# Pointcept/Pointcept

Measured on AMD Instinct MI355X. Metric: scenes/sec (fwd+bwd+optimizer) PTv3 ScanNet-semseg @ ~100k pts, higher is better.
Workload: dtype bf16; 1 GPU; PT-v3m1 base (46.2M params) + seg head + CE + Lovasz, fwd+bwd+AdamW, 8 scenes x 102400 voxels per GPU, patch 1024, 4 orders; global_batch=8, parallelism=dp1, params=46167572, amp=bf16 autocast, points_per_gpu=819200, loss=CrossEntropy(ignore_index=-1) + LovaszSoftmax

## Files before the change

### pointcept_amd/csrc/attention.hip

```cpp
#include "ptc_common.h"
#include <stdlib.h>

typedef __attribute__((ext_vector_type(8))) short s16x8;
typedef __attribute__((ext_vector_type(4))) short s16x4;
typedef __attribute__((ext_vector_type(16))) float f32x16;
typedef __bf16 bf16x2_t __attribute__((ext_vector_type(2)));
typedef float f32x2_t __attribute__((ext_vector_type(2)));

#define AT_WAVES 8
#define AT_THREADS (AT_WAVES * 64)
#define AT_MAX_L 1024
#define AT_MIN_WAVES 4
#define AT_LOG2E 1.4426950408889634f
#define AT_LN2 0.6931471805599453f
#ifndef AT_SPLIT_BELOW
#define AT_SPLIT_BELOW 2048
#endif
#define AT_FIXED_REF_MAX 64.0f

__device__ __forceinline__ uint32_t pack_bf16x2(float lo, float hi) {
  f32x2_t f = {lo, hi};
  bf16x2_t h = __builtin_convertvector(f, bf16x2_t);
  return *reinterpret_cast<uint32_t*>(&h);
}
// ... 389 lines not shown
      if (kt < n_tiles) {
        expo(s1, pb);
        ldv();
        pv(pa);
        ldv();
        pv(pb);
      } else {
        ldv();
        pv(pa);
      }
    } else {
      float m = -INFINITY;
      const unsigned char* kp = kbase;
      const unsigned char* vp = vbase;
      for (int kt = 0; kt < n_tiles; ++kt) {
        const s16x8 kf = *reinterpret_cast<const s16x8*>(kp);
        kp += 1024;
        f32x16 s = mfma32(kf, qhi, zero16());
        s = mfma32(kf, qlo, s);
        if (kt == n_tiles - 1 && L < Lp) {
#pragma unroll
          for (int r = 0; r < 16; ++r)
            if (kt * 32 + crow(r, h2) >= L) s[r] = -INFINITY;
        }
        float mt = s[0];
#pragma unroll
        for (int r = 1; r < 16; ++r) mt = fmaxf(mt, s[r]);
        mt = fmaxf(mt, __shfl_xor(mt, 32, 64));
        const float m_new = fmaxf(m, mt);
        const float alpha = __builtin_amdgcn_exp2f(m - m_new);
        m = m_new;
#pragma unroll
        for (int r = 0; r < 9; ++r) acc[r] *= alpha;
        uint32_t pk[8];
#pragma unroll
        for (int i = 0; i < 8; ++i)
          pk[i] = pack_bf16x2(__builtin_amdgcn_exp2f(s[2 * i] - m), __builtin_amdgcn_exp2f(s[2 * i + 1] - m));
#pragma unroll
        for (int mm = 0; mm < 2; ++mm) {
          const s16x8 pf = make_frag(pk[4 * mm], pk[4 * mm + 1], pk[4 * mm + 2], pk[4 * mm + 3]);
          const s16x8 vf = *reinterpret_cast<const s16x8*>(vp + mm * voff);
          acc = mfma32(vf, pf, acc);
        }
        vp += vstride;
      }
      ref2 = m;
    }
    const float l = __shfl(acc[8], col, 64);
    const float inv = 1.f / l;
    if (q < L) {
      uint16_t* o = out + ((int64_t)(a + q) * H + head) * 16;
      uint2 w0, w1;
      w0.x = at_out<F16>(pack_bf16x2(acc[0] * inv, acc[1] * inv)); w0.y = at_out<F16>(pack_bf16x2(acc[2] * inv, acc[3] * inv));
      w1.x = at_out<F16>(pack_bf16x2(acc[4] * inv, acc[5] * inv)); w1.y = at_out<F16>(pack_bf16x2(acc[6] * inv, acc[7] * inv));
      *reinterpret_cast<uint2*>(o + 4 * h2) = w0;
      *reinterpret_cast<uint2*>(o + 8 + 4 * h2) = w1;
      if (h2 == 0) lse[(int64_t)head * total + a + q] = ref2 * AT_LN2 + __logf(l);
    }
  }
}


__device__ __forceinline__ int at_krow(int g) { return 16 * (g & 1) + 4 * (g >> 1); }
struct TrAddr16 { int lo, hi; };
__device__ __forceinline__ TrAddr16 tr_addr16(int lane) {
  const int lp = lane & 15, g = lane >> 4;
  const int row = at_krow(g) + (lp >> 2), cq = lp & 3;
  TrAddr16 a;
  a.lo = rm_off(row, cq >> 1) + ((cq & 1) << 3);
  a.hi = rm_off(row + 8, cq >> 1) + ((cq & 1) << 3);
  return a;
}
__device__ __forceinline__ void at_to_b16(uint32_t (&pk)[8], s16x8& lo, s16x8& hi) {
#pragma unroll
  for (int j = 0; j < 4; ++j) at_swap16(pk[j], pk[4 + j]);
  lo = make_frag(pk[0], pk[1], pk[2], pk[3]);
  hi = make_frag(pk[4], pk[5], pk[6], pk[7]);
}

template <int LP, bool F16>
__global__ void __launch_bounds__(AT_THREADS, AT_MIN_WAVES)
attn_bwd_dq_kernel(const uint16_t* __restrict__ qkv, const uint16_t* __restrict__ out, const uint16_t* __restrict__ dout,
                   const float* __restrict__ lse, const int32_t* __restrict__ cu, int H, float scale, int64_t total,
                   int lp_max, int n_units, int qs, uint16_t* __restrict__ dqkv, float* __restrict__ delta) {
  extern __shared__ __attribute__((aligned(16))) unsigned char smem[];
  const int lunit = at_unit(n_units * qs);
  if (lunit >= n_units * qs) return;
  const int unit = lunit / qs, part = lunit - unit * qs;
  const int seq = unit / H, head = unit % H;
  const int a = cu[seq], L = cu[seq + 1] - a;
  if (L <= 0) return;
  const int Lp = (L + 31) & ~31, n_tiles = Lp >> 5;
  if (Lp > lp_max) {
    if (part == 0) at_poison_rows<F16>(dqkv + qkv_off(a, 0, H, head), (int64_t)3 * H * 16, L, nullptr);
    return;
  }
  const int t_per = (n_tiles + qs - 1) / qs, t_lo = part * t_per, t_hi = (t_lo + t_per) < n_tiles ? (t_lo + t_per) : n_tiles;
  if (t_lo >= n_tiles) return;
  unsigned char* Vsm = smem;
  unsigned char* Ksm = smem + (size_t)lp_max * 32;
  const int64_t rs = (int64_t)3 * H * 16;
  stage_row_major<F16>(qkv + qkv_off(a, 2, H, head), rs, L, Lp, Vsm);
  stage_row_major<F16>(qkv + qkv_off(a, 1, H, head), rs, L, Lp, Ksm);
  __syncthreads();

  const int lane = ptc_lane(), wave = threadIdx.x >> 6;
  const int col = lane & 31, h2 = lane >> 5;
  const float c = scale * AT_LOG2E;
  const TrAddr16 ta = tr_addr16(lane);
  const int rmo = rm_off(col, h2);

  for (int qt = t_lo + wave; qt < t_hi; qt += AT_WAVES) {
    const int q = qt * 32 + col;
    const bool qv = q < L;
    const s16x8 qf = ld_global_frag<F16>(qkv + qkv_off(a + q, 0, H, head) + h2 * 8, qv);
    const int64_t orow = ((int64_t)(a + q) * H + head) * 16 + h2 * 8;
    const s16x8 dof = ld_global_frag<F16>(dout + orow, qv);
    const s16x8 of = ld_global_frag<F16>(out + orow, qv);
    float dl = 0.f;
#pragma unroll
    for (int j = 0; j < 8; ++j) dl += bf16_bits_to_float((uint16_t)dof[j]) * bf16_bits_to_float((uint16_t)of[j]);
    dl += __shfl_xor(dl, 32, 64);
    const float l2 = qv ? lse[(int64_t)head * total + a + q] * AT_LOG2E : INFINITY;
    if (qv && h2 == 0) delta[(int64_t)head * total + a + q] = dl;
    s16x8 qhi, qlo;
    split_scaled(qf, c, qhi, qlo);
    const f32x16 negl = splat16(-l2), negd = splat16(-dl);
    at_f32x4 acc0 = {0.f, 0.f, 0.f, 0.f}, acc1 = {0.f, 0.f, 0.f, 0.f};
    {
      const int KOFF = LP ? LP * 32 : lp_max * 32;
      const unsigned char* pv = Vsm + rmo;
      const unsigned char* pl = Ksm + ta.lo;
      const unsigned char* ph = Ksm + ta.hi;
      auto tile = [&](const int o) {
        const s16x8 vf = *reinterpret_cast<const s16x8*>(pv + o);
        const s16x8 kf = *reinterpret_cast<const s16x8*>(pv + o + KOFF);
        f32x16 s = mfma32(kf, qhi, negl);
        s = mfma32(kf, qlo, s);
        const f32x16 dp = mfma32(vf, dof, negd);
        uint32_t pk[8];
#pragma unroll
        for (int i = 0; i < 8; ++i)
          pk[i] = pack_bf16x2(__builtin_amdgcn_exp2f(s[2 * i]) * dp[2 * i], __builtin_amdgcn_exp2f(s[2 * i + 1]) * dp[2 * i + 1]);
        s16x8 ds0, ds1;
        at_to_b16(pk, ds0, ds1);
        const s16x8 ktf = ld_tr_pair(pl + o, ph + o);
        acc0 = mfma16(ktf, ds0, acc0);
        acc1 = mfma16(ktf, ds1, acc1);
      };
      int kt = 0;
      for (; kt + 1 < n_tiles; kt += 2) {
        tile(0);
        tile(1024);
        pv += 2048; pl += 2048; ph += 2048;
      }
      if (kt < n_tiles) tile(0);
    }
    const int g = lane >> 4, n = lane & 15;
#pragma unroll
    for (int t = 0; t < 2; ++t) {
      const int qq = qt * 32 + 16 * t + n;
      if (qq < L) {
        const at_f32x4 v = t ? acc1 : acc0;
        uint2 w;
        w.x = at_out<F16>(pack_bf16x2(v[0] * scale, v[1] * scale));
        w.y = at_out<F16>(pack_bf16x2(v[2] * scale, v[3] * scale));
        *reinterpret_cast<uint2*>(dqkv + qkv_off(a + qq, 0, H, head) + 4 * g) = w;
      }
    }
  }
}

#define AT_PAD_LSE 1.0e30f
template <int LP, bool F16>
__global__ void __launch_bounds__(AT_THREADS, AT_MIN_WAVES)
attn_bwd_dkv_kernel(const uint16_t* __restrict__ qkv, const uint16_t* __restrict__ dout, const float* __restrict__ lse,
                    const float* __restrict__ delta, const int32_t* __restrict__ cu, int H, float scale, int64_t total,
                    int lp_max, int n_units, int qs, uint16_t* __restrict__ dqkv) {
  extern __shared__ __attribute__((aligned(16))) unsigned char smem[];
  const int lunit = at_unit(n_units * qs);
  if (lunit >= n_units * qs) return;
  const int unit = lunit / qs, part = lunit - unit * qs;
  const int seq = unit / H, head = unit % H;
  const int a = cu[seq], L = cu[seq + 1] - a;
  if (L <= 0) return;
  const int Lp = (L + 31) & ~31, n_tiles = Lp >> 5;
  if (Lp > lp_max) {
    if (part == 0) {
      at_poison_rows<F16>(dqkv + qkv_off(a, 1, H, head), (int64_t)3 * H * 16, L, nullptr);
      at_poison_rows<F16>(dqkv + qkv_off(a, 2, H, head), (int64_t)3 * H * 16, L, nullptr);
    }
    return;
  }
  const int t_per = (n_tiles + qs - 1) / qs, t_lo = part * t_per, t_hi = (t_lo + t_per) < n_tiles ? (t_lo + t_per) : n_tiles;
  if (t_lo >= n_tiles) return;
  unsigned char* Qsm = smem;
  float* nl = reinterpret_cast<float*>(smem + (size_t)lp_max * 64);
  float* nd = nl + lp_max;
  stage_row_major<F16>(qkv + qkv_off(a, 0, H, head), (int64_t)3 * H * 16, L, Lp, Qsm);
  stage_row_major<F16>(dout + ((int64_t)a * H + head) * 16, (int64_t)H * 16, L, Lp, smem + (size_t)lp_max * 32);
  for (int q = threadIdx.x; q < Lp; q += AT_THREADS) {
    nl[q] = q < L ? -lse[(int64_t)head * total + a + q] * AT_LOG2E : -AT_PAD_LSE;
    nd[q] = q < L ? -delta[(int64_t)head * total + a + q] : 0.f;
  }
  __syncthreads();

  const int lane = ptc_lane(), wave = threadIdx.x >> 6;
  const int col = lane & 31, h2 = lane >> 5;
  const float c = scale * AT_LOG2E;
  const TrAddr16 ta = tr_addr16(lane);
  const int rmo = rm_off(col, h2);

  for (int kt = t_lo + wave; kt < t_hi; kt += AT_WAVES) {
    const int key = kt * 32 + col;
    const s16x8 kf = ld_global_frag<F16>(qkv + qkv_off(a + key, 1, H, head) + h2 * 8, key < L);
    const s16x8 vf = ld_global_frag<F16>(qkv + qkv_off(a + key, 2, H, head) + h2 * 8, key < L);
    s16x8 khi, klo;
    split_scaled(kf, c, khi, klo);
    at_f32x4 dv0 = {0.f, 0.f, 0.f, 0.f}, dv1 = dv0, dk0 = dv0, dk1 = dv0;
    {
      const int DOFF = LP ? LP * 32 : lp_max * 32, NOFF = (LP ? LP : lp_max) * 4;
      const unsigned char* pq = Qsm + rmo;
      const unsigned char* pl = Qsm + ta.lo;
      const unsigned char* ph = Qsm + ta.hi;
      const unsigned char* pc = reinterpret_cast<const unsigned char*>(nl) + 16 * h2;
      auto tile = [&](const int o, const int oc) {
        const s16x8 qf = *reinterpret_cast<const s16x8*>(pq + o);
        const s16x8 dof = *reinterpret_cast<const s16x8*>(pq + o + DOFF);
        f32x16 s, dp;
#pragma unroll
        for (int r4 = 0; r4 < 4; ++r4) {
          const at_f32x4 l4 = *reinterpret_cast<const at_f32x4*>(pc + oc + 32 * r4);
          const at_f32x4 d4 = *reinterpret_cast<const at_f32x4*>(pc + oc + 32 * r4 + NOFF);
#pragma unroll
          for (int e = 0; e < 4; ++e) { s[4 * r4 + e] = l4[e]; dp[4 * r4 + e] = d4[e]; }
        }
        s = mfma32(qf, khi, s);
        s = mfma32(qf, klo, s);
        dp = mfma32(dof, vf, dp);
        uint32_t pp[8], ps[8];
#pragma unroll
        for (int i = 0; i < 8; ++i) {
          const float p0 = __builtin_amdgcn_exp2f(s[2 * i]), p1 = __builtin_amdgcn_exp2f(s[2 * i + 1]);
          pp[i] = pack_bf16x2(p0, p1);
          ps[i] = pack_bf16x2(p0 * dp[2 * i], p1 * dp[2 * i + 1]);
        }
        s16x8 p0f, p1f, s0f, s1f;
        at_to_b16(pp, p0f, p1f);
        at_to_b16(ps, s0f, s1f);
        const s16x8 dotf = ld_tr_pair(pl + o + DOFF, ph + o + DOFF);
        const s16x8 qtf = ld_tr_pair(pl + o, ph + o);
        dv0 = mfma16(dotf, p0f, dv0);
        dv1 = mfma16(dotf, p1f, dv1);
        dk0 = mfma16(qtf, s0f, dk0);
        dk1 = mfma16(qtf, s1f, dk1);
      };
      int qt = 0;
      for (; qt + 1 < n_tiles; qt += 2) {
        tile(0, 0);
        tile(1024, 128);
        pq += 2048; pl += 2048; ph += 2048; pc += 256;
      }
      if (qt < n_tiles) tile(0, 0);
    }
    const int g = lane >> 4, n = lane & 15;
// ... 13 lines not shown
    }
  }
}

#include "attention_bwd1.h"
#include "attention_hd.h"
#include "attention_rpe.h"
#include "attention_rpe_f32.h"
#include "attention_drop.h"

template <typename K>
static int allow_big_lds(K kernel, size_t bytes) {
  PTC_HIP(hipFuncSetAttribute(reinterpret_cast<const void*>(kernel), hipFuncAttributeMaxDynamicSharedMemorySize, (int)bytes));
  return PTC_OK;
}

static size_t fwd_lds_bytes(int lp_max) { return (size_t)lp_max * 32 + (size_t)17 * (lp_max + 8) * 2 + AT_WAVES * 4; }
static size_t at_bwd_pad() { const char* e = getenv("PTC_AT_BWD_PAD_LDS"); return e ? (size_t)atoi(e) : 0; }
static size_t dq_lds_bytes(int lp_max) { return (size_t)lp_max * 64 + at_bwd_pad(); }
static size_t dkv_lds_bytes(int lp_max) { return (size_t)lp_max * 64 + (size_t)lp_max * 8 + at_bwd_pad(); }

static int check_shapes(const char* name, const void* qkv, const int32_t* cu, int64_t n_seq, int64_t total, int H, int max_seqlen);
static int check_common(const char* name, const void* qkv, const int32_t* cu, int64_t n_seq, int64_t total, int H,
                        int max_seqlen, int dtype, bool f16_io = false) {
  PTC_REQUIRE(dtype == PTC_BF16 || (f16_io && dtype == PTC_F16), PTC_EUNSUPPORTED,
              "%s: bf16 arithmetic only (the reference casts qkv to bf16, ptv3m1:209)%s", name, f16_io ? "; tensors bf16 or f16" : "");
  return check_shapes(name, qkv, cu, n_seq, total, H, max_seqlen);
}
static int check_shapes(const char* name, const void* qkv, const int32_t* cu, int64_t n_seq, int64_t total, int H, int max_seqlen) {
  PTC_REQUIRE(n_seq >= 0 && total >= 0 && H >= 1, PTC_EINVAL, "%s: bad sizes", name);
  PTC_REQUIRE(max_seqlen >= 1 && max_seqlen <= AT_MAX_L, PTC_EUNSUPPORTED, "%s: max_seqlen=%d not in [1,%d]", name, max_seqlen, AT_MAX_L);
  PTC_REQUIRE(n_seq * H < (1ll << 29), PTC_EUNSUPPORTED, "%s: grid too large", name);
  PTC_REQUIRE(n_seq == 0 || (qkv && cu), PTC_EINVAL, "%s: null buffer", name);
  PTC_REQUIRE((uintptr_t)qkv % 16 == 0, PTC_EINVAL, "%s: qkv must be 16-byte aligned", name);
  return PTC_OK;
}

extern "C" int ptc_attn_varlen_fwd(const void* qkv, const int32_t* cu_seqlens, int64_t n_seq, int64_t total, int H,
                                   int max_seqlen, float softmax_scale, int dtype, void* out, float* lse,
                                   ptc_stream_t stream) {
  int rc = check_common("ptc_attn_varlen_fwd", qkv, cu_seqlens, n_seq, total, H, max_seqlen, dtype, true);
  if (rc != PTC_OK) return rc;
  if (n_seq == 0 || total == 0) return PTC_OK;
  PTC_REQUIRE(out && lse, PTC_EINVAL, "ptc_attn_varlen_fwd: null buffer");
  const int lp_max = (max_seqlen + 31) & ~31;
  const size_t lds = fwd_lds_bytes(lp_max);
  hipStream_t s = (hipStream_t)stream;
  const int n_units = (int)(n_seq * H);
  const AtPlan plan = at_plan_host(n_units, lp_max);
#define AT_FWD_CASE(F16)                                                                                                                   \
  if ((dtype == PTC_F16) == F16) {                                                                                                          \
    rc = allow_big_lds(attn_fwd_kernel<F16>, lds);                                                                                          \
    if (rc != PTC_OK) return rc;                                                                                                            \
    hipLaunchKernelGGL(attn_fwd_kernel<F16>, dim3((unsigned)(8 * at_plan_blocks_per_xcd(n_units, plan))), dim3(AT_THREADS), lds, s,           \
                       (const uint16_t*)qkv, cu_seqlens, H, softmax_scale, total, lp_max, n_units, plan.qs, plan.whole, (uint16_t*)out, lse); \
    PTC_CHECK_LAUNCH("attn_fwd_kernel");                                                                                                    \
    return PTC_OK;                                                                                                                          \
  }
  AT_FWD_CASE(false) AT_FWD_CASE(true)
#undef AT_FWD_CASE
  return PTC_EINVAL;
}

extern "C" size_t ptc_attn_varlen_bwd_workspace_bytes(int64_t total, int H) {
  return ptc_align_up((size_t)(total > 0 ? total : 1) * (size_t)H * sizeof(float), 256);
}

extern "C" int ptc_attn_varlen_bwd(const void* qkv, const void* out, const void* dout, const float* lse,
                                   const int32_t* cu_seqlens, int64_t n_seq, int64_t total, int H, int max_seqlen,
                                   float softmax_scale, int dtype, void* dqkv, void* workspace, size_t workspace_bytes,
                                   ptc_stream_t stream) {
  int rc = check_common("ptc_attn_varlen_bwd", qkv, cu_seqlens, n_seq, total, H, max_seqlen, dtype, true);
  if (rc != PTC_OK) return rc;
  if (n_seq == 0 || total == 0) return PTC_OK;
  PTC_REQUIRE(out && dout && lse && dqkv && workspace, PTC_EINVAL, "ptc_attn_varlen_bwd: null buffer");
  PTC_REQUIRE(workspace_bytes >= ptc_attn_varlen_bwd_workspace_bytes(total, H), PTC_EWORKSPACE,
              "ptc_attn_varlen_bwd: workspace too small");
  PTC_REQUIRE(((uintptr_t)out % 16 == 0) && ((uintptr_t)dout % 16 == 0) && ((uintptr_t)dqkv % 16 == 0), PTC_EINVAL,
              "ptc_attn_varlen_bwd: buffers must be 16-byte aligned");
  const int lp_max = (max_seqlen + 31) & ~31;
  hipStream_t s = (hipStream_t)stream;
  float* delta = (float*)workspace;
  const int n_units = (int)(n_seq * H);
  {
    const char* e1 = getenv("PTC_AT_BWD1");
    const int forced = e1 ? atoi(e1) : -1;
    if (forced != 0 && lp_max <= AT_MAX_L && (forced == 1 || n_units >= AT1_MIN_UNITS)) {
      const unsigned g1 = (unsigned)(8 * ((n_units + 7) / 8));
#define AT_BWD1_CASE(F16)                                                                                                           \
      if ((dtype == PTC_F16) == F16) {                                                                                              \
        rc = allow_big_lds((attn_bwd1_kernel<F16>), bwd1_lds_bytes(lp_max));                                                        \
        if (rc != PTC_OK) return rc;                                                                                                \
        hipLaunchKernelGGL((attn_bwd1_kernel<F16>), dim3(g1), dim3(AT_THREADS), bwd1_lds_bytes(lp_max), s, (const uint16_t*)qkv,     \
                           (const uint16_t*)out, (const uint16_t*)dout, lse, cu_seqlens, H, softmax_scale, total, lp_max, n_units,  \
                           (uint16_t*)dqkv);                                                                                        \
        PTC_CHECK_LAUNCH("attn_bwd1_kernel");                                                                                       \
        return PTC_OK;                                                                                                              \
      }
      AT_BWD1_CASE(false) AT_BWD1_CASE(true)
#undef AT_BWD1_CASE
    }
  }
  const int qs = at_split_host(n_units, lp_max);
  const unsigned grid = (unsigned)(8 * ((n_units * qs + 7) / 8));
#define AT_BWD_CASE(LP, F16)                                                                                                        \
  if ((LP == 0 ? lp_max != 1024 : lp_max == LP) && (dtype == PTC_F16) == F16) {                                                                                                             \
    rc = allow_big_lds((attn_bwd_dq_kernel<LP, F16>), dq_lds_bytes(lp_max));                                                           \
    if (rc != PTC_OK) return rc;                                                                                               \
    rc = allow_big_lds((attn_bwd_dkv_kernel<LP, F16>), dkv_lds_bytes(lp_max));                                                         \
    if (rc != PTC_OK) return rc;                                                                                               \
    hipLaunchKernelGGL((attn_bwd_dq_kernel<LP, F16>), dim3(grid), dim3(AT_THREADS), dq_lds_bytes(lp_max), s, (const uint16_t*)qkv,     \
                       (const uint16_t*)out, (const uint16_t*)dout, lse, cu_seqlens, H, softmax_scale, total, lp_max, n_units, \
                       qs, (uint16_t*)dqkv, delta);                                                                            \
    PTC_CHECK_LAUNCH("attn_bwd_dq_kernel");                                                                                    \
    hipLaunchKernelGGL((attn_bwd_dkv_kernel<LP, F16>), dim3(grid), dim3(AT_THREADS), dkv_lds_bytes(lp_max), s, (const uint16_t*)qkv,   \
                       (const uint16_t*)dout, lse, (const float*)delta, cu_seqlens, H, softmax_scale, total, lp_max, n_units,  \
                       qs, (uint16_t*)dqkv);                                                                                   \
    PTC_CHECK_LAUNCH("attn_bwd_dkv_kernel");                                                                                   \
    return PTC_OK;                                                                                                             \
  }
  AT_BWD_CASE(1024, false) AT_BWD_CASE(0, false) AT_BWD_CASE(1024, true) AT_BWD_CASE(0, true)
#undef AT_BWD_CASE
  return PTC_EINVAL;
}

static int drop_params(const char* name, float p, uint32_t* thresh, float* rp) {
  PTC_REQUIRE(p >= 0.f && p < 1.f, PTC_EINVAL, "%s: dropout_p=%g must lie in [0, 1)", name, (double)p);
  const double t = (double)p * 4294967296.0;
  *thresh = t >= 4294967295.0 ? 0xFFFFFFFFu : (uint32_t)t;
  *rp = 1.f / (1.f - p);
  return PTC_OK;
}

extern "C" int ptc_attn_varlen_dropout_fwd(const void* qkv, const int32_t* cu_seqlens, int64_t n_seq, int64_t total, int H, int max_seqlen,
                                           float softmax_scale, int dtype, float dropout_p, uint64_t seed, void* out, float* lse,
                                           ptc_stream_t stream) {
  int rc = check_common("ptc_attn_varlen_dropout_fwd", qkv, cu_seqlens, n_seq, total, H, max_seqlen, dtype, true);
  if (rc != PTC_OK) return rc;
  uint32_t thresh;
  float rp;
  rc = drop_params("ptc_attn_varlen_dropout_fwd", dropout_p, &thresh, &rp);
  if (rc != PTC_OK) return rc;
  if (n_seq == 0 || total == 0) return PTC_OK;
  PTC_REQUIRE(out && lse, PTC_EINVAL, "ptc_attn_varlen_dropout_fwd: null buffer");
  const int lp_max = (max_seqlen + 31) & ~31;
  const size_t lds = fwd_lds_bytes(lp_max);
  const int n_units = (int)(n_seq * H);
  const unsigned grid = (unsigned)(8 * ((n_units + 7) / 8));
#define AD_FWD_CASE(F16)                                                                                                             \
  if ((dtype == PTC_F16) == F16) {                                                                                                   \
    rc = allow_big_lds(attn_drop_fwd_kernel<F16>, lds);                                                                              \
    if (rc != PTC_OK) return rc;                                                                                                     \
    hipLaunchKernelGGL(attn_drop_fwd_kernel<F16>, dim3(grid), dim3(AT_THREADS), lds, (hipStream_t)stream, (const uint16_t*)qkv,      \
                       cu_seqlens, H, softmax_scale, total, lp_max, n_units, thresh, rp, (uint32_t)seed, (uint32_t)(seed >> 32),     \
                       (uint16_t*)out, lse);                                                                                         \
    PTC_CHECK_LAUNCH("attn_drop_fwd_kernel");                                                                                        \
    return PTC_OK;                                                                                                                   \
  }
  AD_FWD_CASE(false) AD_FWD_CASE(true)
#undef AD_FWD_CASE
  return PTC_EINVAL;
}

extern "C" int ptc_attn_varlen_dropout_bwd(const void* qkv, const void* out, const void* dout, const float* lse, const int32_t* cu_seqlens,
                                           int64_t n_seq, int64_t total, int H, int max_seqlen, float softmax_scale, int dtype,
                                           float dropout_p, uint64_t seed, void* dqkv, void* workspace, size_t workspace_bytes,
                                           ptc_stream_t stream) {
  int rc = check_common("ptc_attn_varlen_dropout_bwd", qkv, cu_seqlens, n_seq, total, H, max_seqlen, dtype, true);
  if (rc != PTC_OK) return rc;
  uint32_t thresh;
  float rp;
  rc = drop_params("ptc_attn_varlen_dropout_bwd", dropout_p, &thresh, &rp);
  if (rc != PTC_OK) return rc;
  if (n_seq == 0 || total == 0) return PTC_OK;
  PTC_REQUIRE(out && dout && lse && dqkv && workspace, PTC_EINVAL, "ptc_attn_varlen_dropout_bwd: null buffer");
  PTC_REQUIRE(workspace_bytes >= ptc_attn_varlen_bwd_workspace_bytes(total, H), PTC_EWORKSPACE, "ptc_attn_varlen_dropout_bwd: workspace too small");
  PTC_REQUIRE(((uintptr_t)out % 16 == 0) && ((uintptr_t)dout % 16 == 0) && ((uintptr_t)dqkv % 16 == 0), PTC_EINVAL,
              "ptc_attn_varlen_dropout_bwd: buffers must be 16-byte aligned");
  const int lp_max = (max_seqlen + 31) & ~31;
  hipStream_t s = (hipStream_t)stream;
  float* delta = (float*)workspace;
  const int n_units = (int)(n_seq * H);
  const unsigned grid = (unsigned)(8 * ((n_units + 7) / 8));
  const size_t lds_q = (size_t)lp_max * 64, lds_kv = (size_t)lp_max * 64 + (size_t)lp_max * 8;
#define AD_BWD_CASE(F16)                                                                                                             \
  if ((dtype == PTC_F16) == F16) {                                                                                                   \
    rc = allow_big_lds(attn_drop_bwd_dq_kernel<F16>, lds_q);                                                                         \
    if (rc != PTC_OK) return rc;                                                                                                     \
    rc = allow_big_lds(attn_drop_bwd_dkv_kernel<F16>, lds_kv);                                                                       \
    if (rc != PTC_OK) return rc;                                                                                                     \
    hipLaunchKernelGGL(attn_drop_bwd_dq_kernel<F16>, dim3(grid), dim3(AT_THREADS), lds_q, s, (const uint16_t*)qkv, (const uint16_t*)out, \
                       (const uint16_t*)dout, lse, cu_seqlens, H, softmax_scale, total, lp_max, n_units, thresh, rp, (uint32_t)seed, \
                       (uint32_t)(seed >> 32), (uint16_t*)dqkv, delta);                                                              \
    PTC_CHECK_LAUNCH("attn_drop_bwd_dq_kernel");                                                                                     \
    hipLaunchKernelGGL(attn_drop_bwd_dkv_kernel<F16>, dim3(grid), dim3(AT_THREADS), lds_kv, s, (const uint16_t*)qkv,                 \
                       (const uint16_t*)dout, lse, (const float*)delta, cu_seqlens, H, softmax_scale, total, lp_max, n_units, thresh, \
                       rp, (uint32_t)seed, (uint32_t)(seed >> 32), (uint16_t*)dqkv);                                                 \
    PTC_CHECK_LAUNCH("attn_drop_bwd_dkv_kernel");                                                                                    \
    return PTC_OK;                                                                                                                   \
  }
// ... 294 lines not shown
```

### pointcept_amd/csrc/attention_bwd1.h

```cpp
#pragma once

#define AT1_KT 4
#ifndef AT1_MIN_UNITS
#define AT1_MIN_UNITS 176
#endif
#define AT1_SLICE 2048
#ifndef AT1_PIPE
#define AT1_PIPE 1
#endif
static size_t bwd1_lds_bytes(int lp_max) { return (size_t)lp_max * 72 + (size_t)AT_WAVES * AT1_SLICE * 4; }

__device__ __forceinline__ int at1_ds_off(int key, int c) { return key * 64 + ((c ^ ((key >> 1) & 7)) << 3); }

template <bool F16>
__global__ void __launch_bounds__(AT_THREADS, 2)
attn_bwd1_kernel(const uint16_t* __restrict__ qkv, const uint16_t* __restrict__ out, const uint16_t* __restrict__ dout,
                 const float* __restrict__ lse, const int32_t* __restrict__ cu, int H, float scale, int64_t total, int lp_max, int n_units,
                 uint16_t* __restrict__ dqkv) {
  extern __shared__ __attribute__((aligned(16))) unsigned char smem[];
  const int unit = at_unit(n_units);
  if (unit >= n_units) return;
  const int seq = unit / H, head = unit % H;
  const int a = cu[seq], L = cu[seq + 1] - a;
  if (L <= 0) return;
  const int Lp = (L + 31) & ~31, n_tiles = Lp >> 5;
  const int64_t rs = (int64_t)3 * H * 16;
  if (Lp > lp_max) {
    for (int j = 0; j < 3; ++j) at_poison_rows<F16>(dqkv + qkv_off(a, j, H, head), rs, L, nullptr);
    return;
  }
  unsigned char* Qsm = smem;
  unsigned char* Dsm = smem + (size_t)lp_max * 32;
  float* nl = reinterpret_cast<float*>(smem + (size_t)lp_max * 64);
  float* nd = nl + lp_max;
  const int lane = ptc_lane(), wave = threadIdx.x >> 6;
  unsigned char* slice = smem + (size_t)lp_max * 72 + (size_t)wave * (2 * AT1_SLICE);
  unsigned char* red = smem + (size_t)lp_max * 72 + (size_t)AT_WAVES * (2 * AT1_SLICE);

  stage_row_major<F16>(qkv + qkv_off(a, 0, H, head), rs, L, Lp, Qsm);
  for (int row = threadIdx.x; row < Lp; row += AT_THREADS) {
    uint4 d0 = {0, 0, 0, 0}, d1 = d0, o0 = d0, o1 = d0;
    float l2 = AT_PAD_LSE;
    if (row < L) {
      const int64_t orow = ((int64_t)(a + row) * H + head) * 16;
      const uint4* pd = reinterpret_cast<const uint4*>(dout + orow);
      const uint4* po = reinterpret_cast<const uint4*>(out + orow);
      d0 = at_in<F16>(pd[0]); d1 = at_in<F16>(pd[1]);
      o0 = at_in<F16>(po[0]); o1 = at_in<F16>(po[1]);
      l2 = lse[(int64_t)head * total + a + row] * AT_LOG2E;
    }
    *reinterpret_cast<uint4*>(Dsm + rm_off(row, 0)) = d0;
    *reinterpret_cast<uint4*>(Dsm + rm_off(row, 1)) = d1;
    const uint32_t wd[8] = {d0.x, d0.y, d0.z, d0.w, d1.x, d1.y, d1.z, d1.w}, wo[8] = {o0.x, o0.y, o0.z, o0.w, o1.x, o1.y, o1.z, o1.w};
    float dl[2] = {0.f, 0.f};
#pragma unroll
    for (int j = 0; j < 8; ++j) {
      dl[j >> 2] += __uint_as_float(wd[j] << 16) * __uint_as_float(wo[j] << 16);
      dl[j >> 2] += __uint_as_float(wd[j] & 0xffff0000u) * __uint_as_float(wo[j] & 0xffff0000u);
    }
    nl[row] = -l2;
    nd[row] = -(dl[0] + dl[1]);
  }

  const int col = lane & 31, h2 = lane >> 5;
  const int g = lane >> 4, n = lane & 15;
  const float c = scale * AT_LOG2E;
  const TrAddr16 ta = tr_addr16(lane);
  const int rmo = rm_off(col, h2);
  const int n_own = n_tiles > wave ? (n_tiles - wave + AT_WAVES - 1) / AT_WAVES : 0;

  s16x8 khi[AT1_KT], klo[AT1_KT], vf[AT1_KT], kta[AT1_KT];
  at_f32x4 dk0[AT1_KT], dk1[AT1_KT], dv0[AT1_KT], dv1[AT1_KT];
#pragma unroll
  for (int j = 0; j < AT1_KT; ++j) {
    const at_f32x4 z = {0.f, 0.f, 0.f, 0.f};
    dk0[j] = dk1[j] = dv0[j] = dv1[j] = z;
    const int kt = wave + AT_WAVES * j;
    const int key = kt * 32 + col;
    const bool kv = j < n_own && key < L;
    const s16x8 kf = ld_global_frag<F16>(qkv + qkv_off(a + key, 1, H, head) + h2 * 8, kv);
    vf[j] = ld_global_frag<F16>(qkv + qkv_off(a + key, 2, H, head) + h2 * 8, kv);
    split_scaled(kf, c, khi[j], klo[j]);
    uint32_t w[4];
#pragma unroll
    for (int e = 0; e < 4; ++e) {
      uint32_t two = 0;
#pragma unroll
      for (int b = 0; b < 2; ++b) {
        const int k2 = kt * 32 + 8 * g + 2 * e + b;
        uint32_t v = 0;
        if (j < n_own && k2 < L) {
          v = qkv[qkv_off(a + k2, 1, H, head) + n];
          if constexpr (F16) v = at_f16x2_to_bf16x2(v) & 0xffffu;
        }
        two |= v << (16 * b);
      }
      w[e] = two;
    }
    kta[j] = make_frag(w[0], w[1], w[2], w[3]);
  }
  int wr[4], rd[2][2];
#pragma unroll
  for (int r4 = 0; r4 < 4; ++r4) wr[r4] = at1_ds_off(col, 2 * r4 + h2);
#pragma unroll
  for (int t = 0; t < 2; ++t) {
    rd[t][0] = at1_ds_off(8 * g + (n >> 2), 4 * t + (n & 3));
    rd[t][1] = at1_ds_off(8 * g + 4 + (n >> 2), 4 * t + (n & 3));
  }
  __syncthreads();

  s16x8 qf, dof, qtf, dotf;
  f32x16 cl, cd;
  auto load_q_tile = [&](int qt) {
    const int o = qt * 1024;
    qf = *reinterpret_cast<const s16x8*>(Qsm + rmo + o);
    dof = *reinterpret_cast<const s16x8*>(Dsm + rmo + o);
    qtf = ld_tr_pair(Qsm + ta.lo + o, Qsm + ta.hi + o);
    dotf = ld_tr_pair(Dsm + ta.lo + o, Dsm + ta.hi + o);
#pragma unroll
    for (int r4 = 0; r4 < 4; ++r4) {
      const at_f32x4 l4 = *reinterpret_cast<const at_f32x4*>(nl + qt * 32 + 8 * r4 + 4 * h2);
      const at_f32x4 d4 = *reinterpret_cast<const at_f32x4*>(nd + qt * 32 + 8 * r4 + 4 * h2);
#pragma unroll
      for (int e = 0; e < 4; ++e) { cl[4 * r4 + e] = l4[e]; cd[4 * r4 + e] = d4[e]; }
    }
  };
  for (int qt = 0; qt < n_tiles; ++qt) {
    load_q_tile(qt);
    at_f32x4 acc0 = {0.f, 0.f, 0.f, 0.f}, acc1 = acc0;
    if (AT1_PIPE && n_own == AT1_KT) {
      s16x8 b0 = qf, b1 = qf;
#pragma unroll
      for (int j = 0; j <= AT1_KT; ++j) {
        f32x16 s, dp;
        if (j < AT1_KT) {
          s = mfma32(qf, khi[j], cl);
          s = mfma32(qf, klo[j], s);
          dp = mfma32(dof, vf[j], cd);
        }
        if (j > 0) {
          __builtin_amdgcn_fence(__ATOMIC_RELEASE, "wavefront");
          __builtin_amdgcn_wave_barrier();
          __builtin_amdgcn_fence(__ATOMIC_ACQUIRE, "wavefront");
          const unsigned char* sl = slice + ((j - 1) & 1) * AT1_SLICE;
          b0 = ld_tr_pair(sl + rd[0][0], sl + rd[0][1]);
          b1 = ld_tr_pair(sl + rd[1][0], sl + rd[1][1]);
        }
        if (j < AT1_KT) {
          uint32_t pp[8], ps[8];
#pragma unroll
          for (int i = 0; i < 8; ++i) {
            const float p0 = __builtin_amdgcn_exp2f(s[2 * i]), p1 = __builtin_amdgcn_exp2f(s[2 * i + 1]);
            pp[i] = pack_bf16x2(p0, p1);
            ps[i] = pack_bf16x2(p0 * dp[2 * i], p1 * dp[2 * i + 1]);
          }
#pragma unroll
          for (int r4 = 0; r4 < 4; ++r4)
            *reinterpret_cast<uint2*>(slice + (j & 1) * AT1_SLICE + wr[r4]) = make_uint2(ps[2 * r4], ps[2 * r4 + 1]);
          s16x8 p0f, p1f, s0f, s1f;
          at_to_b16(pp, p0f, p1f);
          at_to_b16(ps, s0f, s1f);
          dv0[j] = mfma16(dotf, p0f, dv0[j]);
          dv1[j] = mfma16(dotf, p1f, dv1[j]);
          dk0[j] = mfma16(qtf, s0f, dk0[j]);
          dk1[j] = mfma16(qtf, s1f, dk1[j]);
        }
        if (j > 0) {
          acc0 = mfma16(kta[j - 1], b0, acc0);
          acc1 = mfma16(kta[j - 1], b1, acc1);
        }
      }
    } else {
#pragma unroll
    for (int j = 0; j < AT1_KT; ++j) {
      if (j < n_own) {
        f32x16 s = mfma32(qf, khi[j], cl);
        s = mfma32(qf, klo[j], s);
        const f32x16 dp = mfma32(dof, vf[j], cd);
        uint32_t pp[8], ps[8];
#pragma unroll
        for (int i = 0; i < 8; ++i) {
          const float p0 = __builtin_amdgcn_exp2f(s[2 * i]), p1 = __builtin_amdgcn_exp2f(s[2 * i + 1]);
          pp[i] = pack_bf16x2(p0, p1);
          ps[i] = pack_bf16x2(p0 * dp[2 * i], p1 * dp[2 * i + 1]);
        }
#pragma unroll
        for (int r4 = 0; r4 < 4; ++r4) *reinterpret_cast<uint2*>(slice + wr[r4]) = make_uint2(ps[2 * r4], ps[2 * r4 + 1]);
        s16x8 p0f, p1f, s0f, s1f;
        at_to_b16(pp, p0f, p1f);
        at_to_b16(ps, s0f, s1f);
        dv0[j] = mfma16(dotf, p0f, dv0[j]);
        dv1[j] = mfma16(dotf, p1f, dv1[j]);
        dk0[j] = mfma16(qtf, s0f, dk0[j]);
        dk1[j] = mfma16(qtf, s1f, dk1[j]);
        __builtin_amdgcn_fence(__ATOMIC_RELEASE, "wavefront");
        __builtin_amdgcn_wave_barrier();
        __builtin_amdgcn_fence(__ATOMIC_ACQUIRE, "wavefront");
        const s16x8 b0 = ld_tr_pair(slice + rd[0][0], slice + rd[0][1]);
        const s16x8 b1 = ld_tr_pair(slice + rd[1][0], slice + rd[1][1]);
        acc0 = mfma16(kta[j], b0, acc0);
        acc1 = mfma16(kta[j], b1, acc1);
        __builtin_amdgcn_fence(__ATOMIC_RELEASE, "wavefront");
        __builtin_amdgcn_wave_barrier();
        __builtin_amdgcn_fence(__ATOMIC_ACQUIRE, "wavefront");
      }
    }
    }
    unsigned char* rp = red + (size_t)((qt & 1) * AT_WAVES + wave) * AT1_SLICE;
    *reinterpret_cast<at_f32x4*>(rp + n * 64 + ((g ^ (n & 3)) << 4)) = acc0;
    *reinterpret_cast<at_f32x4*>(rp + (16 + n) * 64 + ((g ^ (n & 3)) << 4)) = acc1;
    __syncthreads();
    if ((wave >> 1) == (qt & 3)) {
      const int t2 = (wave & 1) * 64 + lane, q = t2 >> 2, d4 = t2 & 3;
      const unsigned char* r0 = red + (size_t)((qt & 1) * AT_WAVES) * AT1_SLICE + q * 64 + ((d4 ^ (q & 3)) << 4);
      at_f32x4 sum = *reinterpret_cast<const at_f32x4*>(r0);
#pragma unroll
      for (int w = 1; w < AT_WAVES; ++w) {
        const at_f32x4 v = *reinterpret_cast<const at_f32x4*>(r0 + w * AT1_SLICE);
#pragma unroll
        for (int e = 0; e < 4; ++e) sum[e] += v[e];
      }
      const int qq = qt * 32 + q;
      if (qq < L) {
        uint2 w2;
        w2.x = at_out<F16>(pack_bf16x2(sum[0] * scale, sum[1] * scale));
        w2.y = at_out<F16>(pack_bf16x2(sum[2] * scale, sum[3] * scale));
        *reinterpret_cast<uint2*>(dqkv + qkv_off(a + qq, 0, H, head) + 4 * d4) = w2;
      }
    }
  }
#pragma unroll
  for (int j = 0; j < AT1_KT; ++j) {
    if (j >= n_own) continue;
    const int kt = wave + AT_WAVES * j;
#pragma unroll
    for (int t = 0; t < 2; ++t) {
      const int kk = kt * 32 + 16 * t + n;
      if (kk < L) {
        const at_f32x4 vk = t ? dk1[j] : dk0[j], vv = t ? dv1[j] : dv0[j];
        uint2 wk, wv;
        wk.x = at_out<F16>(pack_bf16x2(vk[0] * scale, vk[1] * scale));
        wk.y = at_out<F16>(pack_bf16x2(vk[2] * scale, vk[3] * scale));
        wv.x = at_out<F16>(pack_bf16x2(vv[0], vv[1]));
        wv.y = at_out<F16>(pack_bf16x2(vv[2], vv[3]));
        *reinterpret_cast<uint2*>(dqkv + qkv_off(a + kk, 1, H, head) + 4 * g) = wk;
        *reinterpret_cast<uint2*>(dqkv + qkv_off(a + kk, 2, H, head) + 4 * g) = wv;
      }
    }
  }
}
```

Baseline: 232.8 scenes/s.

## Split fused attention backward into full-wave pass plus split-dQ tail pass

Plans the fused single-kernel attention backward so that whole multiples of the CU count run in the fused kernel. The leftover tail units get a dQ-only variant of the fused kernel, split across query tiles, which also writes delta. The split dK/dV kernel then handles only the tail units. This targets the wave-quantization imbalance where a small remainder of units would otherwise occupy a nearly empty last wave, at the cost of extra launches and some recomputation of the score matrix for the tail units.

New measurement: 230.9 scenes/s. About the same (-0.8%).

```diff
diff --git a/pointcept_amd/csrc/attention.hip b/pointcept_amd/csrc/attention.hip
--- a/pointcept_amd/csrc/attention.hip
+++ b/pointcept_amd/csrc/attention.hip
@@ -495,11 +495,11 @@
 __global__ void __launch_bounds__(AT_THREADS, AT_MIN_WAVES)
 attn_bwd_dq_kernel(const uint16_t* __restrict__ qkv, const uint16_t* __restrict__ out, const uint16_t* __restrict__ dout,
                    const float* __restrict__ lse, const int32_t* __restrict__ cu, int H, float scale, int64_t total,
-                   int lp_max, int n_units, int qs, uint16_t* __restrict__ dqkv, float* __restrict__ delta) {
+                   int lp_max, int n_units, int unit_lo, int qs, uint16_t* __restrict__ dqkv, float* __restrict__ delta) {
   extern __shared__ __attribute__((aligned(16))) unsigned char smem[];
   const int lunit = at_unit(n_units * qs);
   if (lunit >= n_units * qs) return;
-  const int unit = lunit / qs, part = lunit - unit * qs;
+  const int unit = unit_lo + lunit / qs, part = lunit % qs;
   const int seq = unit / H, head = unit % H;
   const int a = cu[seq], L = cu[seq + 1] - a;
   if (L <= 0) return;
@@ -589,11 +589,11 @@
 __global__ void __launch_bounds__(AT_THREADS, AT_MIN_WAVES)
 attn_bwd_dkv_kernel(const uint16_t* __restrict__ qkv, const uint16_t* __restrict__ dout, const float* __restrict__ lse,
                     const float* __restrict__ delta, const int32_t* __restrict__ cu, int H, float scale, int64_t total,
-                    int lp_max, int n_units, int qs, uint16_t* __restrict__ dqkv) {
+                    int lp_max, int n_units, int unit_lo, int qs, uint16_t* __restrict__ dqkv) {
   extern __shared__ __attribute__((aligned(16))) unsigned char smem[];
   const int lunit = at_unit(n_units * qs);
   if (lunit >= n_units * qs) return;
-  const int unit = lunit / qs, part = lunit - unit * qs;
+  const int unit = unit_lo + lunit / qs, part = lunit % qs;
   const int seq = unit / H, head = unit % H;
   const int a = cu[seq], L = cu[seq + 1] - a;
   if (L <= 0) return;
@@ -773,40 +773,56 @@
   hipStream_t s = (hipStream_t)stream;
   float* delta = (float*)workspace;
   const int n_units = (int)(n_seq * H);
+  int split_lo = 0, split_n = n_units;
+  bool split_dq = true;
   {
     const char* e1 = getenv("PTC_AT_BWD1");
     const int forced = e1 ? atoi(e1) : -1;
     if (forced != 0 && lp_max <= AT_MAX_L && (forced == 1 || n_units >= AT1_MIN_UNITS)) {
-      const unsigned g1 = (unsigned)(8 * ((n_units + 7) / 8));
+      const At1Plan plan = at1_plan_host(n_units);
+      const unsigned g1 = (unsigned)(8 * ((plan.full + 7) / 8)), gt = (unsigned)(8 * ((plan.tail * plan.qs + 7) / 8));
 #define AT_BWD1_CASE(F16)                                                                                                           \
       if ((dtype == PTC_F16) == F16) {                                                                                              \
-        rc = allow_big_lds((attn_bwd1_kernel<F16>), bwd1_lds_bytes(lp_max));                                                        \
-        if (rc != PTC_OK) return rc;                                                                                                \
-        hipLaunchKernelGGL((attn_bwd1_kernel<F16>), dim3(g1), dim3(AT_THREADS), bwd1_lds_bytes(lp_max), s, (const uint16_t*)qkv,     \
-                           (const uint16_t*)out, (const uint16_t*)dout, lse, cu_seqlens, H, softmax_scale, total, lp_max, n_units,  \
-                           (uint16_t*)dqkv);                                                                                        \
-        PTC_CHECK_LAUNCH("attn_bwd1_kernel");                                                                                       \
-        return PTC_OK;                                                                                                              \
+        if (plan.full > 0) {                                                                                                        \
+          rc = allow_big_lds((attn_bwd1_kernel<F16, false>), bwd1_lds_bytes(lp_max));                                               \
+          if (rc != PTC_OK) return rc;                                                                                              \
+          hipLaunchKernelGGL((attn_bwd1_kernel<F16, false>), dim3(g1), dim3(AT_THREADS), bwd1_lds_bytes(lp_max), s,                 \
+                             (const uint16_t*)qkv, (const uint16_t*)out, (const uint16_t*)dout, lse, cu_seqlens, H, softmax_scale,  \
+                             total, lp_max, plan.full, 0, 1, (uint16_t*)dqkv, (float*)nullptr);                                     \
+          PTC_CHECK_LAUNCH("attn_bwd1_kernel");                                                                                     \
+        }                                                                                                                           \
+        if (plan.tail > 0) {                                                                                                        \
+          rc = allow_big_lds((attn_bwd1_kernel<F16, true>), bwd1_lds_bytes(lp_max));                                                \
+          if (rc != PTC_OK) return rc;                                                                                              \
+          hipLaunchKernelGGL((attn_bwd1_kernel<F16, true>), dim3(gt), dim3(AT_THREADS), bwd1_lds_bytes(lp_max), s,                  \
+                             (const uint16_t*)qkv, (const uint16_t*)out, (const uint16_t*)dout, lse, cu_seqlens, H, softmax_scale,  \
+                             total, lp_max, plan.tail, plan.full, plan.qs, (uint16_t*)dqkv, delta);                                 \
+          PTC_CHECK_LAUNCH("attn_bwd1_kernel (tail dQ)");                                                                           \
+        }                                                                                                                           \
       }
       AT_BWD1_CASE(false) AT_BWD1_CASE(true)
 #undef AT_BWD1_CASE
-    }
-  }
-  const int qs = at_split_host(n_units, lp_max);
-  const unsigned grid = (unsigned)(8 * ((n_units * qs + 7) / 8));
+      if (plan.tail == 0) return PTC_OK;
+      split_lo = plan.full; split_n = plan.tail; split_dq = false;
+    }
+  }
+  const int qs = at_split_host(split_n, lp_max);
+  const unsigned grid = (unsigned)(8 * ((split_n * qs + 7) / 8));
 #define AT_BWD_CASE(LP, F16)                                                                                                        \
   if ((LP == 0 ? lp_max != 1024 : lp_max == LP) && (dtype == PTC_F16) == F16) {                                                                                                             \
     rc = allow_big_lds((attn_bwd_dq_kernel<LP, F16>), dq_lds_bytes(lp_max));                                                           \
     if (rc != PTC_OK) return rc;                                                                                               \
     rc = allow_big_lds((attn_bwd_dkv_kernel<LP, F16>), dkv_lds_bytes(lp_max));                                                         \
     if (rc != PTC_OK) return rc;                                                                                               \
-    hipLaunchKernelGGL((attn_bwd_dq_kernel<LP, F16>), dim3(grid), dim3(AT_THREADS), dq_lds_bytes(lp_max), s, (const uint16_t*)qkv,     \
-                       (const uint16_t*)out, (const uint16_t*)dout, lse, cu_seqlens, H, softmax_scale, total, lp_max, n_units, \
-                       qs, (uint16_t*)dqkv, delta);                                                                            \
-    PTC_CHECK_LAUNCH("attn_bwd_dq_kernel");                                                                                    \
+    if (split_dq) {                                                                                                            \
+      hipLaunchKernelGGL((attn_bwd_dq_kernel<LP, F16>), dim3(grid), dim3(AT_THREADS), dq_lds_bytes(lp_max), s, (const uint16_t*)qkv,   \
+                         (const uint16_t*)out, (const uint16_t*)dout, lse, cu_seqlens, H, softmax_scale, total, lp_max, split_n, \
+                         split_lo, qs, (uint16_t*)dqkv, delta);                                                                \
+      PTC_CHECK_LAUNCH("attn_bwd_dq_kernel");                                                                                  \
+    }                                                                                                                          \
     hipLaunchKernelGGL((attn_bwd_dkv_kernel<LP, F16>), dim3(grid), dim3(AT_THREADS), dkv_lds_bytes(lp_max), s, (const uint16_t*)qkv,   \
-                       (const uint16_t*)dout, lse, (const float*)delta, cu_seqlens, H, softmax_scale, total, lp_max, n_units,  \
-                       qs, (uint16_t*)dqkv);                                                                                   \
+                       (const uint16_t*)dout, lse, (const float*)delta, cu_seqlens, H, softmax_scale, total, lp_max, split_n,  \
+                       split_lo, qs, (uint16_t*)dqkv);                                                                         \
     PTC_CHECK_LAUNCH("attn_bwd_dkv_kernel");                                                                                   \
     return PTC_OK;                                                                                                             \
   }
diff --git a/pointcept_amd/csrc/attention_bwd1.h b/pointcept_amd/csrc/attention_bwd1.h
--- a/pointcept_amd/csrc/attention_bwd1.h
+++ b/pointcept_amd/csrc/attention_bwd1.h
@@ -3,6 +3,9 @@
 #define AT1_KT 4
 #ifndef AT1_MIN_UNITS
 #define AT1_MIN_UNITS 176
+#endif
+#ifndef AT1_TAIL_MAX_UNITS
+#define AT1_TAIL_MAX_UNITS 128
 #endif
 #define AT1_SLICE 2048
 #ifndef AT1_PIPE
@@ -10,25 +13,60 @@
 #endif
 static size_t bwd1_lds_bytes(int lp_max) { return (size_t)lp_max * 72 + (size_t)AT_WAVES * AT1_SLICE * 4; }
 
+struct At1Plan { int full, tail, qs; };
+static int at1_slots() {
+  if (const char* e = getenv("PTC_AT_BWD_SLOTS")) { const int v = atoi(e); if (v > 0) return v; }
+#ifdef __HIPCC__
+  static int cached[64] = {0};
+  int dev = 0;
+  if (hipGetDevice(&dev) != hipSuccess || dev < 0 || dev >= 64) return 256;
+  if (cached[dev] <= 0) {
+    int n = 0;
+    cached[dev] = (hipDeviceGetAttribute(&n, hipDeviceAttributeMultiprocessorCount, dev) == hipSuccess && n > 0) ? n : 256;
+  }
+  return cached[dev];
+#else
+  return 256;
+#endif
+}
+static At1Plan at1_plan_host(int n_units) {
+  const char* e = getenv("PTC_AT_BWD_PLAN");
+  const int mode = e ? atoi(e) : 1;
+  const int slots = at1_slots();
+  At1Plan p = {n_units, 0, 1};
+  if (mode == 2) p = {0, n_units, 1};
+  else if (mode != 0) {
+    const int full = (n_units / slots) * slots, rem = n_units - full;
+    if (full > 0 && rem > 0 && (long long)rem * 256 <= (long long)AT1_TAIL_MAX_UNITS * slots) p = {full, rem, 1};
+  }
+  while (p.tail > 0 && p.qs < 8 && p.tail * p.qs < slots) p.qs *= 2;
+  return p;
+}
+
 __device__ __forceinline__ int at1_ds_off(int key, int c) { return key * 64 + ((c ^ ((key >> 1) & 7)) << 3); }
 
-template <bool F16>
+template <bool F16, bool DQ>
 __global__ void __launch_bounds__(AT_THREADS, 2)
 attn_bwd1_kernel(const uint16_t* __restrict__ qkv, const uint16_t* __restrict__ out, const uint16_t* __restrict__ dout,
                  const float* __restrict__ lse, const int32_t* __restrict__ cu, int H, float scale, int64_t total, int lp_max, int n_units,
-                 uint16_t* __restrict__ dqkv) {
+                 int unit_lo, int qs, uint16_t* __restrict__ dqkv, float* __restrict__ delta) {
   extern __shared__ __attribute__((aligned(16))) unsigned char smem[];
-  const int unit = at_unit(n_units);
-  if (unit >= n_units) return;
+  const int lunit = at_unit(DQ ? n_units * qs : n_units);
+  if (lunit >= (DQ ? n_units * qs : n_units)) return;
+  const int unit = unit_lo + (DQ ? lunit / qs : lunit), part = DQ ? lunit % qs : 0;
   const int seq = unit / H, head = unit % H;
   const int a = cu[seq], L = cu[seq + 1] - a;
   if (L <= 0) return;
   const int Lp = (L + 31) & ~31, n_tiles = Lp >> 5;
   const int64_t rs = (int64_t)3 * H * 16;
   if (Lp > lp_max) {
-    for (int j = 0; j < 3; ++j) at_poison_rows<F16>(dqkv + qkv_off(a, j, H, head), rs, L, nullptr);
+    if (part == 0)
+      for (int j = 0; j < (DQ ? 1 : 3); ++j) at_poison_rows<F16>(dqkv + qkv_off(a, j, H, head), rs, L, nullptr);
     return;
   }
+  const int t_per = DQ ? (n_tiles + qs - 1) / qs : n_tiles;
+  const int t_lo = part * t_per, t_hi = (t_lo + t_per) < n_tiles ? (t_lo + t_per) : n_tiles;
+  if (t_lo >= n_tiles) return;
   unsigned char* Qsm = smem;
   unsigned char* Dsm = smem + (size_t)lp_max * 32;
   float* nl = reinterpret_cast<float*>(smem + (size_t)lp_max * 64);
@@ -37,9 +75,9 @@
   unsigned char* slice = smem + (size_t)lp_max * 72 + (size_t)wave * (2 * AT1_SLICE);
   unsigned char* red = smem + (size_t)lp_max * 72 + (size_t)AT_WAVES * (2 * AT1_SLICE);
 
-  stage_row_major<F16>(qkv + qkv_off(a, 0, H, head), rs, L, Lp, Qsm);
-  for (int row = threadIdx.x; row < Lp; row += AT_THREADS) {
-    uint4 d0 = {0, 0, 0, 0}, d1 = d0, o0 = d0, o1 = d0;
+  if constexpr (!DQ) stage_row_major<F16>(qkv + qkv_off(a, 0, H, head), rs, L, Lp, Qsm);
+  for (int row = t_lo * 32 + threadIdx.x; row < t_hi * 32; row += AT_THREADS) {
+    uint4 d0 = {0, 0, 0, 0}, d1 = d0, o0 = d0, o1 = d0, q0 = d0, q1 = d0;
     float l2 = AT_PAD_LSE;
     if (row < L) {
       const int64_t orow = ((int64_t)(a + row) * H + head) * 16;
@@ -48,6 +86,14 @@
       d0 = at_in<F16>(pd[0]); d1 = at_in<F16>(pd[1]);
       o0 = at_in<F16>(po[0]); o1 = at_in<F16>(po[1]);
       l2 = lse[(int64_t)head * total + a + row] * AT_LOG2E;
+      if constexpr (DQ) {
+        const uint4* pq = reinterpret_cast<const uint4*>(qkv + qkv_off(a + row, 0, H, head));
+        q0 = at_in<F16>(pq[0]); q1 = at_in<F16>(pq[1]);
+      }
+    }
+    if constexpr (DQ) {
+      *reinterpret_cast<uint4*>(Qsm + rm_off(row, 0)) = q0;
+      *reinterpret_cast<uint4*>(Qsm + rm_off(row, 1)) = q1;
     }
     *reinterpret_cast<uint4*>(Dsm + rm_off(row, 0)) = d0;
     *reinterpret_cast<uint4*>(Dsm + rm_off(row, 1)) = d1;
@@ -60,6 +106,9 @@
     }
     nl[row] = -l2;
     nd[row] = -(dl[0] + dl[1]);
+    if constexpr (DQ) {
+      if (row < L) delta[(int64_t)head * total + a + row] = dl[0] + dl[1];
+    }
   }
 
   const int col = lane & 31, h2 = lane >> 5;
@@ -115,8 +164,10 @@
     const int o = qt * 1024;
     qf = *reinterpret_cast<const s16x8*>(Qsm + rmo + o);
     dof = *reinterpret_cast<const s16x8*>(Dsm + rmo + o);
-    qtf = ld_tr_pair(Qsm + ta.lo + o, Qsm + ta.hi + o);
-    dotf = ld_tr_pair(Dsm + ta.lo + o, Dsm + ta.hi + o);
+    if constexpr (!DQ) {
+      qtf = ld_tr_pair(Qsm + ta.lo + o, Qsm + ta.hi + o);
+      dotf = ld_tr_pair(Dsm + ta.lo + o, Dsm + ta.hi + o);
+    }
 #pragma unroll
     for (int r4 = 0; r4 < 4; ++r4) {
       const at_f32x4 l4 = *reinterpret_cast<const at_f32x4*>(nl + qt * 32 + 8 * r4 + 4 * h2);
@@ -125,7 +176,7 @@
       for (int e = 0; e < 4; ++e) { cl[4 * r4 + e] = l4[e]; cd[4 * r4 + e] = d4[e]; }
     }
   };
-  for (int qt = 0; qt < n_tiles; ++qt) {
+  for (int qt = t_lo; qt < t_hi; ++qt) {
     load_q_tile(qt);
     at_f32x4 acc0 = {0.f, 0.f, 0.f, 0.f}, acc1 = acc0;
     if (AT1_PIPE && n_own == AT1_KT) {
@@ -157,6 +208,38 @@
 #pragma unroll
           for (int r4 = 0; r4 < 4; ++r4)
             *reinterpret_cast<uint2*>(slice + (j & 1) * AT1_SLICE + wr[r4]) = make_uint2(ps[2 * r4], ps[2 * r4 + 1]);
+          if constexpr (!DQ) {
+            s16x8 p0f, p1f, s0f, s1f;
+            at_to_b16(pp, p0f, p1f);
+            at_to_b16(ps, s0f, s1f);
+            dv0[j] = mfma16(dotf, p0f, dv0[j]);
+            dv1[j] = mfma16(dotf, p1f, dv1[j]);
+            dk0[j] = mfma16(qtf, s0f, dk0[j]);
+            dk1[j] = mfma16(qtf, s1f, dk1[j]);
+          }
+        }
+        if (j > 0) {
+          acc0 = mfma16(kta[j - 1], b0, acc0);
+          acc1 = mfma16(kta[j - 1], b1, acc1);
+        }
+      }
+    } else {
+#pragma unroll
+    for (int j = 0; j < AT1_KT; ++j) {
+      if (j < n_own) {
+        f32x16 s = mfma32(qf, khi[j], cl);
+        s = mfma32(qf, klo[j], s);
+        const f32x16 dp = mfma32(dof, vf[j], cd);
+        uint32_t pp[8], ps[8];
+#pragma unroll
+        for (int i = 0; i < 8; ++i) {
+          const float p0 = __builtin_amdgcn_exp2f(s[2 * i]), p1 = __builtin_amdgcn_exp2f(s[2 * i + 1]);
+          pp[i] = pack_bf16x2(p0, p1);
+          ps[i] = pack_bf16x2(p0 * dp[2 * i], p1 * dp[2 * i + 1]);
+        }
+#pragma unroll
+        for (int r4 = 0; r4 < 4; ++r4) *reinterpret_cast<uint2*>(slice + wr[r4]) = make_uint2(ps[2 * r4], ps[2 * r4 + 1]);
+        if constexpr (!DQ) {
           s16x8 p0f, p1f, s0f, s1f;
           at_to_b16(pp, p0f, p1f);
           at_to_b16(ps, s0f, s1f);
@@ -165,34 +248,6 @@
           dk0[j] = mfma16(qtf, s0f, dk0[j]);
           dk1[j] = mfma16(qtf, s1f, dk1[j]);
         }
-        if (j > 0) {
-          acc0 = mfma16(kta[j - 1], b0, acc0);
-          acc1 = mfma16(kta[j - 1], b1, acc1);
-        }
-      }
-    } else {
-#pragma unroll
-    for (int j = 0; j < AT1_KT; ++j) {
-      if (j < n_own) {
-        f32x16 s = mfma32(qf, khi[j], cl);
-        s = mfma32(qf, klo[j], s);
-        const f32x16 dp = mfma32(dof, vf[j], cd);
-        uint32_t pp[8], ps[8];
-#pragma unroll
-        for (int i = 0; i < 8; ++i) {
-          const float p0 = __builtin_amdgcn_exp2f(s[2 * i]), p1 = __builtin_amdgcn_exp2f(s[2 * i + 1]);
-          pp[i] = pack_bf16x2(p0, p1);
-          ps[i] = pack_bf16x2(p0 * dp[2 * i], p1 * dp[2 * i + 1]);
-        }
-#pragma unroll
-        for (int r4 = 0; r4 < 4; ++r4) *reinterpret_cast<uint2*>(slice + wr[r4]) = make_uint2(ps[2 * r4], ps[2 * r4 + 1]);
-        s16x8 p0f, p1f, s0f, s1f;
-        at_to_b16(pp, p0f, p1f);
-        at_to_b16(ps, s0f, s1f);
-        dv0[j] = mfma16(dotf, p0f, dv0[j]);
-        dv1[j] = mfma16(dotf, p1f, dv1[j]);
-        dk0[j] = mfma16(qtf, s0f, dk0[j]);
-        dk1[j] = mfma16(qtf, s1f, dk1[j]);
         __builtin_amdgcn_fence(__ATOMIC_RELEASE, "wavefront");
         __builtin_amdgcn_wave_barrier();
         __builtin_amdgcn_fence(__ATOMIC_ACQUIRE, "wavefront");
@@ -229,6 +284,7 @@
       }
     }
   }
+  if constexpr (DQ) return;
 #pragma unroll
   for (int j = 0; j < AT1_KT; ++j) {
     if (j >= n_own) continue;
```
